# aras-p/ToyPathTracer

Measured on AMD Instinct MI355X. Metric: Mray/s, higher is better.
Workload: dtype f32

## Files before the change

include/tpt_test_hooks.h:

```cpp
#ifndef TPT_TEST_HOOKS_H
#define TPT_TEST_HOOKS_H
#include "tpt_hip.h"
#ifdef __cplusplus
extern "C" {
#endif
TPT_API int tptTestMath(int op, const float* a, const float* b, float* out, int n);
TPT_API int tptTestHitSpheres(int hitSpheres, const float* rays, int* outId, float* outT, int n);
TPT_API int tptTestMathExhaustive(int op, unsigned lo, unsigned hi, unsigned long long* outMismatches, unsigned* outFirst8);
TPT_API int tptTestMatrixFilter(const float* rays, unsigned long long* outMask, int* outId, float* outT, int n);
TPT_API int tptTestGroupFilter(const float* rays, int n, unsigned long long* outViolations, unsigned long long* outTouched, unsigned long long* outExact);
TPT_API int tptTestSetDealCapacities(int superGroupEntries, int groupEntries, int survivorEntries);
TPT_API int tptDebugStats(unsigned long long* out128, int reset);
TPT_API int tptDebugChunkOrder(unsigned* outCost, unsigned* outOrder, int capacity);
#ifdef __cplusplus
}
#endif
#endif
```

toypathtracer_amd/api.py:

```python
import ctypes as C
import os

import numpy as np

kFlagAnimate = 1 << 0
kFlagProgressive = 1 << 1
SEED_ROW_SERIAL, SEED_PER_PIXEL = 0, 1
FOLD_RECURSIVE, FOLD_FORWARD = 0, 1

SPHERE_DT = np.dtype([("cx", "<f4"), ("cy", "<f4"), ("cz", "<f4"), ("radius", "<f4"), ("invRadius", "<f4")])
MATERIAL_DT = np.dtype([("type", "<i4"), ("albedo", "<f4", 3), ("emissive", "<f4", 3), ("roughness", "<f4"), ("ri", "<f4")])
CAMERA_DT = np.dtype([("origin", "<f4", 3), ("lowerLeftCorner", "<f4", 3), ("horizontal", "<f4", 3), ("vertical", "<f4", 3),
                      ("uu", "<f4", 3), ("vv", "<f4", 3), ("ww", "<f4", 3), ("lensRadius", "<f4")])


class TptError(RuntimeError):
    pass


_lib = None
_product = None
_hooks = None

C_ABI_SYMBOLS = [
    "tptInitialize", "tptShutdown", "tptUpdate", "tptDraw", "tptGetObjectCount", "tptGetSceneDesc",
    "tptSetSamplesPerPixel", "tptSetConfig", "tptSetSeedMode", "tptSetFoldMode", "tptSetScene", "tptSetCamera", "tptSetStream",
    "tptSetRowShard", "tptLocalRowCount", "tptLocalRowToGlobal", "tptDrawDevice", "tptRayCounterRead", "tptSetRayCounter", "tptSetFrameOverlap", "tptDisplayRGBA8", "tptKernelTimingBegin", "tptKernelTimingEnd",
    "tptSynchronize", "tptTimerBegin", "tptTimerEnd", "tptSetKernelVariant",
    "tptDrawDeviceBatch", "tptDrawDeviceViews", "tptDrawDeviceAnimation", "tptDrawDeviceAov", "tptDenoiseDevice", "tptDrawDeviceMoments", "tptDrawDeviceAnimationMoments", "tptDrawDeviceCameraClip", "tptDrawDeviceKeyframeClip", "tptDenoiseDeviceVariance", "tptTemporalAccumulateDevice", "tptObjectPlaneDevice", "tptObjectMotionTable", "tptTemporalAccumulateObjectsDevice", "tptDenoiseClipDevice", "tptMotionVectorsDevice", "tptRectifyHistoryDevice", "tptDrawDeviceAdaptive", "tptAdaptiveSamplesDevice", "tptDrawShardedBatch", "tptGetLookaheadHits", "tptCommGetUniqueId", "tptCommInit", "tptCommInitLoopback", "tptCommInfo", "tptCommDestroy", "tptDrawSharded", "tptSetShardExchangeInterval", "tptShardedFinish", "tptGetLaunchInfo", "tptGetPipelineInfo", "tptGetSceneInfo", "tptSetHostBufferMode", "tptSetHostLookahead", "tptSetStreamBatching", "tptSetTileMirror", "tptGetLastError", "tptSetErrorHandler", "tptGetDeviceName",
]
HOOK_SYMBOLS = ["tptTestMath", "tptTestMathExhaustive", "tptTestHitSpheres", "tptTestMatrixFilter", "tptTestGroupFilter", "tptTestSetDealCapacities", "tptDebugStats", "tptDebugChunkOrder"]
CXX_ABI_SYMBOLS = [
    "_Z14InitializeTestv", "_Z12ShutdownTestv", "_Z10UpdateTestfiiij", "_Z8DrawTestfiiiPfRij",
    "_Z14GetObjectCountRiS_S_S_", "_Z12GetSceneDescPvS_S_S_Pi",
]


class ClipDenoiseArgs(C.Structure):
    _fields_ = ([("screenWidth", C.c_int), ("screenHeight", C.c_int), ("nFrames", C.c_int), ("clipFlags", C.c_uint)]
                + [(name, C.c_void_p) for name in ("deviceFrameImages", "deviceFrameMoments", "deviceFrameAlbedo", "deviceFrameNormalDepth",
                                                   "cameras", "deviceFrameObjects", "deviceFrameObjectMotion", "deviceFrameOut",
                                                   "prevCamera", "devicePrevNormalDepth", "devicePrevObject", "deviceHistory")]
                + [("nObjects", C.c_int), ("iterations", C.c_int), ("denoiseFlags", C.c_uint)]
                + [(name, C.c_float) for name in ("samples", "sigmaLuminance", "sigmaNormal", "sigmaDepth", "maxHistory", "depthTolerance",
                                                  "normalTolerance", "coverageTolerance")])


class MotionVectorsArgs(C.Structure):
    _fields_ = ([("screenWidth", C.c_int), ("screenHeight", C.c_int), ("nFrames", C.c_int), ("flags", C.c_uint)]
                + [(name, C.c_void_p) for name in ("cameras", "deviceFrameAlbedo", "deviceFrameNormalDepth", "deviceFrameObjects",
                                                   "deviceFrameObjectMotion", "deviceFrameMotion", "prevCamera", "devicePrevAlbedo",
                                                   "devicePrevNormalDepth", "devicePrevObject")]
                + [("nObjects", C.c_int)]
                + [(name, C.c_float) for name in ("depthTolerance", "normalTolerance", "coverageTolerance")])


def _lib_dir():
    return os.environ.get("TPT_LIB_DIR") or os.path.join(os.path.dirname(os.path.abspath(__file__)), "lib")


def library_path():
    return os.environ.get("TPT_LIB") or os.path.join(_lib_dir(), "libtoypathtracer_hip.so")


def hooks_library_path():
    return os.environ.get("TPT_LIB") or os.path.join(_lib_dir(), "libtoypathtracer_hip_hooks.so")


def _bind(path, hooks):
    lib = C.CDLL(path)
    i, f, u, p = C.c_int, C.c_float, C.c_uint, C.c_void_p
    sigs = {
        "tptInitialize": [], "tptShutdown": [], "tptUpdate": [f, i, i, i, u],
        "tptDraw": [f, i, i, i, p, C.POINTER(i), u],
        "tptGetObjectCount": [C.POINTER(i)] * 4, "tptGetSceneDesc": [p, p, p, p, C.POINTER(i)],
        "tptSetSamplesPerPixel": [i], "tptSetConfig": [i, f, i], "tptSetSeedMode": [i], "tptSetFoldMode": [i], "tptSetScene": [p, p, i],
        "tptSetCamera": [p, p, f, f, f], "tptSetStream": [p], "tptSetRowShard": [i, i, i], "tptLocalRowCount": [i],
        "tptLocalRowToGlobal": [i], "tptDrawDevice": [f, i, i, i, p, u], "tptRayCounterRead": [C.POINTER(C.c_int64)],
        "tptSetRayCounter": [p], "tptSetTileMirror": [p, p], "tptSetFrameOverlap": [i], "tptDisplayRGBA8": [p, i, i, p], "tptKernelTimingBegin": [i],
        "tptKernelTimingEnd": [C.POINTER(f), C.POINTER(i)],
        "tptSynchronize": [], "tptTimerBegin": [], "tptTimerEnd": [C.POINTER(f)], "tptSetKernelVariant": [i, i, i],
        "tptGetLaunchInfo": [C.POINTER(i)] * 4, "tptGetPipelineInfo": [C.POINTER(i)] * 4, "tptGetSceneInfo": [C.POINTER(i)] * 3, "tptCommGetUniqueId": [p], "tptCommInit": [p, i, i, i], "tptCommInitLoopback": [i, i], "tptCommInfo": [C.POINTER(i)] * 3, "tptCommDestroy": [], "tptDrawSharded": [f, i, i, i, p, u], "tptSetShardExchangeInterval": [i], "tptDrawShardedBatch": [f, i, i, i, i, p, u], "tptDrawDeviceBatch": [f, i, i, i, i, p, u], "tptDrawDeviceViews": [f, i, i, i, i, p, p, p, u], "tptDrawDeviceAnimation": [i, i, p, i, i, p, p, p, u], "tptDrawDeviceAov": [f, i, i, i, p, p, p, u], "tptDenoiseDevice": [i, i, p, p, p, p, i, f, f, f, u], "tptDrawDeviceMoments": [f, i, i, i, p, p, p, p, u], "tptDrawDeviceAnimationMoments": [i, i, p, i, i] + [p] * 7 + [u], "tptDrawDeviceCameraClip": [i, i, p, p, i, i] + [p] * 8 + [u], "tptDrawDeviceKeyframeClip": [i, i, p, i, p, p, i, i] + [p] * 9 + [u], "tptDenoiseDeviceVariance": [i, i, p, p, p, p, f, p, i, f, f, f, u], "tptTemporalAccumulateDevice": [i, i] + [p] * 14 + [f] * 4, "tptObjectPlaneDevice": [i, p, p, i, i, p, u], "tptObjectMotionTable": [f, f, u, p, i], "tptTemporalAccumulateObjectsDevice": [i, i] + [p] * 14 + [f] * 4 + [p, p, p, i], "tptDenoiseClipDevice": [C.POINTER(ClipDenoiseArgs)], "tptMotionVectorsDevice": [C.POINTER(MotionVectorsArgs)], "tptRectifyHistoryDevice": [i, i] + [p] * 7 + [i, f], "tptDrawDeviceAdaptive": [f, i, i, i, p, p, p, p, p, u], "tptAdaptiveSamplesDevice": [i, i, p, f, i, i, p, p, p], "tptShardedFinish": [C.POINTER(C.c_int64)], "tptSetHostBufferMode": [i], "tptGetLookaheadHits": [C.POINTER(C.c_longlong)], "tptSetHostLookahead": [i], "tptSetStreamBatching": [i],
    }
    if hooks:
        sigs.update({"tptDebugStats": [p, i], "tptDebugChunkOrder": [p, p, i], "tptTestMath": [i, p, p, p, i], "tptTestMathExhaustive": [i, u, u, p, p],
                     "tptTestHitSpheres": [i, p, p, p, i], "tptTestMatrixFilter": [p, p, p, p, i], "tptTestGroupFilter": [p, i, p, p, p], "tptTestSetDealCapacities": [i, i, i]})
    for name, args in sigs.items():
        fn = getattr(lib, name)
        fn.argtypes = args
        fn.restype = i
    lib.tptGetLastError.restype = C.c_char_p
    lib.tptGetDeviceName.restype = C.c_char_p
    return lib


def _preload():
    try:
        import torch
    except ImportError:
        pass


def load_library():
    global _lib, _product
    if _lib is not None:
        return _lib
    _preload()
    path = library_path()
    if not os.path.exists(path):
        raise TptError(f"{path} is missing: build it with `python -c 'import __graft_entry__ as g; g.build()'` "
                       "(toypathtracer_amd/csrc/build.sh). There is no CPU fallback.")
    _product = _bind(path, hooks=bool(os.environ.get("TPT_LIB")) and _has_hooks(path))
    _lib = _product
    return _lib


def _has_hooks(path):
    try:
        return hasattr(C.CDLL(path), "tptTestMath")
# ... 835 lines not shown


def test_hit_spheres(rays, hit_spheres=0):
    rays = np.ascontiguousarray(rays, np.float32).reshape(-1, 6)
    n = rays.shape[0]
    ids = np.empty(n, np.int32)
    ts = np.empty(n, np.float32)
    _chk(_hook("tptTestHitSpheres")(hit_spheres, rays.ctypes.data, ids.ctypes.data, ts.ctypes.data, n),
         "tptTestHitSpheres")
    return ids, ts


def test_matrix_filter(rays, hits=False):
    rays = np.ascontiguousarray(rays, np.float32).reshape(-1, 6)
    n = rays.shape[0]
    masks = np.empty(n, np.uint64)
    ids = np.empty(n, np.int32) if hits else None
    ts = np.empty(n, np.float32) if hits else None
    _chk(_hook("tptTestMatrixFilter")(rays.ctypes.data, masks.ctypes.data, ids.ctypes.data if hits else None,
                                            ts.ctypes.data if hits else None, n), "tptTestMatrixFilter")
    return (masks, ids, ts) if hits else masks


def test_set_deal_capacities(super_group_entries=0, group_entries=0, survivor_entries=0):
    _chk(_hook("tptTestSetDealCapacities")(super_group_entries, group_entries, survivor_entries), "tptTestSetDealCapacities")


def test_group_filter(rays):
    rays = np.ascontiguousarray(rays, np.float32).reshape(-1, 6)
    n = rays.shape[0]
    v = [C.c_ulonglong(0) for _ in range(3)]
    _chk(_hook("tptTestGroupFilter")(rays.ctypes.data, n, C.byref(v[0]), C.byref(v[1]), C.byref(v[2])), "tptTestGroupFilter")
    return int(v[0].value), v[1].value / n, v[2].value / n
```

toypathtracer_amd/csrc/tpt_context.h:

```cpp
#pragma once
#include "../../include/tpt_hip.h"
#if defined(TPT_TEST_HOOKS)
#include "../../include/tpt_test_hooks.h"
#endif
#include "../../include/tpt_test_api.h"
#include "tpt_device.h"
#include "tpt_queue_layout.h"
#include "tpt_scene.h"
#include "tpt_shard.h"
#include "tpt_stream_batch.h"
#include "tpt_animation.h"
#include <hip/hip_runtime.h>
#include <thread>
#include <rccl/rccl.h>
#include <chrono>
#include <dlfcn.h>
#include <map>
#include <stdio.h>
#include <stdlib.h>
#include <string>


namespace tpth {
using namespace tpt;

const int kMaxBatch = 32;
static_assert(kMaxBatch == TPT_Q_VIEWS_MAX, "a batch's cameras, centres and ray counts have their places in the path-queue kernel's LDS");
struct TraceTicket {
    int slot = 0, nPixels = 0;
    bool pipelined = false, valid = false;
    float lerpFac = 0;
    const f4* colour = nullptr;
    int batch = 1;
    tptLerpTable lerp = {};
    const f4* moments = nullptr;
    TraceTicket plane(int j) const
    {
        TraceTicket t = *this;
        t.colour = colour + (size_t)j * (size_t)nPixels;
        if (batch > 1) t.lerpFac = lerp.v[j];
        t.batch = 1;
        return t;
    }
};

struct Streak {
    int frame = 0, w = 0, h = 0, n = 0;
    unsigned flags = 0;
    unsigned long long key = 0;
    int next(int frame_, int w_, int h_, unsigned flags_, unsigned long long key_)
    {
        n = frame_ == frame + 1 && w_ == w && h_ == h && flags_ == flags && key_ == key ? n + 1 : 0;
        frame = frame_; w = w_; h = h_; flags = flags_; key = key_;
        return n;
    }
};

struct PendingLaunch {
    enum Kind { AHEAD, ROW_SERIAL, STREAM } kind = AHEAD;
    TraceTicket T;
    int firstFrame = 0, next = 0;
    int w = 0, h = 0;
    unsigned flags = 0;
    unsigned long long key = 0;
    unsigned long long* rays = nullptr;
};
struct LaunchQueue {
    static const int kCap = 4;
    PendingLaunch e[kCap];
    int n = 0;
    bool empty() const { return n == 0; }
    bool holds(PendingLaunch::Kind kind) const { return n > 0 && e[0].kind == kind; }
    bool frontMatches(PendingLaunch::Kind kind, int frame, int w, int h, unsigned flags, unsigned long long key) const;
    void serveFront(bool wasOpen, TraceTicket& T, const unsigned long long*& rays);
    int push(const PendingLaunch& L);
    int discard();
    void closeStream();
};

struct Context {
    static const int kMaxOverlap = 16;
    static const int kMaxSlots = 2 * kMaxOverlap;
    static const int kOrderTables = kMaxSlots + 2;
    bool inited = false;
    int device = 0, numCUs = 0;
    int traceCUs = 0;
    std::string deviceName, err;
    hipStream_t ownStream = nullptr, stream = nullptr;
    hipEvent_t ev0 = nullptr, ev1 = nullptr;

    std::vector<SpherePOD> spheres;
    std::vector<MaterialPOD> mats;
    CameraSetup camSetup = defaultCameraSetup();
    CameraPOD cam;
    PackedScene packed;
    bool sceneDirty = true;
    bool updated = false;
    int updatedW = 0, updatedH = 0;

    static const int kSceneSets = 2 * kMaxSlots;
    struct SceneSet {
        char* dev = nullptr;
        char* stage = nullptr;
        size_t cap = 0, bytes = 0;
        size_t offSph4 = 0, offInvR = 0, offMats = 0, offLights = 0;
        size_t offGPairs = 0, offGSph = 0, offGId = 0, offBSph = 0, offBId = 0;
        size_t offSPairs = 0;
        int nSuperPairs = 0;
        size_t offAmat = 0;
        int mxR1 = -1;
// ... 34 lines not shown
    long long lastTotal = 0;

    f4* dStack[kMaxSlots] = {};
    size_t stackCap = 0, colourCap = 0;
    int slotsReserved = 0;
    int smallStreak = 0;
    int slotReservations = 0;
    unsigned* dChunkCost = nullptr;
    unsigned* dChunkOrder[kOrderTables] = {};
    unsigned* dChunkSnap[kMaxOverlap] = {};
    int chunkCap = 0, chunkCount = 0;
    int costOrder = 1;
    hipEvent_t evOrder = nullptr;
    hipStream_t orderStream = nullptr;
    unsigned long long orderSeq = 0;
    int lastOrderTable = 0;
    float* dFrame = nullptr;
    hipStream_t hostStream2 = nullptr;
    hipEvent_t evBand = nullptr, evBandEnd = nullptr;
    int hostTrust = 0;
    const float* tileSrc = nullptr;
    int tileW = 0, tileH = 0;
    int lookahead = 2;
    LaunchQueue pending;
    struct HostCaller {
        Streak seq;
        int refusedW = 0, refusedH = 0;
        unsigned long long refusedKey = 0;
    } hostCaller;
    static const int kStreamBatchMax = 8, kStreamRing = 64;
    unsigned long long streamBatches = 0;
    int streamRun = 0, streamNext = -1;
    int streamBatch = 1;
    struct DeviceCaller {
        int lastSlot = -1, syncStreak = 0;
        Streak seq;
    } devCaller;
    struct ViewSlot {
        CameraPOD* dev = nullptr;
        unsigned long long* rays = nullptr;
        CameraPOD* stage = nullptr;
        hipEvent_t evUploaded = nullptr;
        bool copyEnqueued = false;
    } views[kMaxSlots];
    char* dViews = nullptr;
    CameraPOD* hViewsStage = nullptr;
    f4* dAovSums = nullptr;
    size_t aovSumsBytes = 0;
    hipEvent_t evAov = nullptr;
    f4* dMoments = nullptr;
    size_t momentsBytes = 0;
    hipEvent_t evClip[2] = {nullptr, nullptr};
    unsigned clipSeq = 0;
    f4* dKeySph = nullptr;
    f4* hKeySph = nullptr;
    size_t keySphBytes = 0;
    hipEvent_t evKeySph[2] = {nullptr, nullptr};
    bool keySphCopied[2] = {false, false};
    unsigned keySphSeq = 0;
    f4* dDenoise = nullptr;
    size_t denoiseBytes = 0;
    f4* dClipStage = nullptr;
    size_t clipStageBytes = 0;
    tptFlowConsts* dFlowConsts = nullptr;
    tptFlowConsts* hFlowConsts = nullptr;
    size_t flowConstsBytes = 0;
// ... 145 lines not shown
```

toypathtracer_amd/csrc/tpt_device.h:

```cpp
#pragma once
#include "tpt_trace.h"
#include "tpt_frame_pools.h"

#ifndef TPT_BLOCK
#define TPT_BLOCK 64
#endif
#define TPT_CHUNK_PIXELS 256

namespace tpt {

struct KernelArgs {
    SceneView scene;
    FrameConsts fc;
    f4* frameColour;
    int nLocalRows, stripeRows, stripeStride, stripeOffset;
    int tilesX;
    int numItems;
    int numChunks, chunkSize;
    int batchFrames, chunksPerFrame, framePlane;
    unsigned totalWaves;
    int laneCap;
    int noRefill;
    f4* stackBuf;
    int stackStride;
    int ldsStackLevels;
    f4* pathBuf;
    const unsigned* chunkOrder;
    unsigned* chunkCost;
    int chunkShift;
    unsigned* work;
    unsigned long long* rayCounter;
    int rayCounterStride;
    unsigned gen;
    int helperBase;
    int helperPct;
    int ldsGroupPairs;
    const CameraPOD* viewCams = nullptr;
    const f4* moveCentres = nullptr;
    f4* aovSums = nullptr;
    f4* aovAlbedo = nullptr;
    f4* aovNormalDepth = nullptr;
    f4* momentsOut = nullptr;
    int aovPlane = 0;
    const int32_t* sampleCounts = nullptr;
    const f4* keyCentres = nullptr;
    unsigned long long keyMask = 0;
    int keyCount = 0;
    int framePools = 0;
};

}

hipError_t tptLaunchTrace(const tpt::KernelArgs& a, int hs, int fold, bool ldsScene, int blocks, size_t lds, hipStream_t stream);
int tptTraceOccupancy(int hs, int fold, bool ldsScene, size_t lds);
hipError_t tptLaunchTraceQueue(const tpt::KernelArgs& a, bool ldsScene, int blocks, size_t lds, hipStream_t stream);
int tptQueueMatrixFilter();
int tptQueueGroupMatrixBounds();
hipError_t tptLaunchDisplay(const float* tile, unsigned char* rgba, int width, int height, hipStream_t stream);
__attribute__((weak)) hipError_t tptLaunchDenoise(const float* colour, const float* albedo, const float* normalDepth, float* out,
                                                  float* scratch, int width, int height, int iterations, float ic, float in, float id,
                                                  bool demodulate, hipStream_t stream);
__attribute__((weak)) hipError_t tptLaunchDenoiseVariance(const float* colour, const float* albedo, const float* normalDepth,
                                                          const float* moments, float* out, float* scratch, int width, int height,
                                                          int iterations, float samples, float sl2, float in, float id, bool demodulate,
                                                          hipStream_t stream);
__attribute__((weak)) hipError_t tptLaunchFramesAtrous(const float* colour, const float* albedo, const float* normalDepth,
                                                       const float* moments, float* out, float* scratch, int width, int height, int frames,
                                                       int iterations, float samples, float sl2, float in, float id, bool demodulate,
                                                       hipStream_t stream);
struct tptTemporalConsts {
    float o[3], ll[3], H[3], V[3];
    float po[3], pa[3], pw[3], pH[3], pV[3];
    float pf, phh, pvv;
    float maxHistory, depthTol, normalTol, coverageTol;
};
__attribute__((weak)) hipError_t tptLaunchTemporal(const float* colour, const float* albedo, const float* normalDepth, const float* moments,
                                                   const float* prevColour, const float* prevAlbedo, const float* prevNormalDepth,
                                                   const float* prevMoments, float* outColour, float* outAlbedo, float* outMoments,
                                                   float* outVariance, int width, int height, const tptTemporalConsts& k,
                                                   hipStream_t stream);
struct tptObjectPlaneConsts {
// ... 53 lines not shown
```

toypathtracer_amd/csrc/tpt_frame_pools.h:

```cpp
#pragma once

#if defined(__HIPCC__)
#define TPT_FP_HD __host__ __device__ inline
#else
#define TPT_FP_HD inline
#endif

namespace tpt {

const int kFramePoolBase = 4;
const int kFramePoolsMax = 8;

TPT_FP_HD int framePoolsOfLaunch(int batch, int blocks, bool plain, bool helpable)
{
    return (plain && !helpable && batch >= 2 && batch <= kFramePoolsMax && blocks >= 2 * batch) ? batch : 0;
}

TPT_FP_HD unsigned framePoolOfBlock(unsigned block, unsigned pools, unsigned blocks)
{
    return block * pools / blocks;
}

}
```

toypathtracer_amd/csrc/tpt_host.cpp:

```cpp
#include "tpt_context.h"

using namespace tpt;
using namespace tpth;

namespace tpth {

Context g;

int localRows(int h) { return shardLocalRows(h, g.stripeRows, g.numParts, g.part); }
int localToGlobal(int ly) { return shardLocalToGlobal(ly, g.stripeRows, g.numParts, g.part); }

template <class T>
int ensureDev(T*& p, int& cap, int need)
{
    if (need <= cap && p) return 0;
    if (p) HIPCHK(hipFree(p));
    p = nullptr;
    int n = need < 64 ? 64 : need;
    HIPCHK(hipMalloc(reinterpret_cast<void**>(&p), sizeof(T) * (size_t)n));
    cap = n;
    return 0;
}

size_t align256(size_t v) { return (v + 255) & ~(size_t)255; }
// ... 249 lines not shown
    hipDeviceProp_t prop;
    HIPCHK(hipGetDeviceProperties(&prop, dev));
    g.device = dev;
    g.numCUs = prop.multiProcessorCount;
    g.deviceName = std::string(prop.name) + " (" + prop.gcnArchName + ")";
    HIPCHK(hipStreamCreateWithFlags(&g.ownStream, hipStreamDefault));
    g.stream = g.ownStream;
    HIPCHK(hipEventCreateWithFlags(&g.evOrder, kOrderingEvent));
    HIPCHK(hipEventCreate(&g.ev0));
    HIPCHK(hipEventCreate(&g.ev1));
    HIPCHK(hipMalloc(reinterpret_cast<void**>(&g.dWork), 64 * Context::kMaxSlots));
    HIPCHK(hipMemsetAsync(g.dWork, 0, 64 * Context::kMaxSlots, g.stream));
    {
        int rc = createTraceStreams();
        if (rc) return rc;
    }
    for (int k = 0; k < Context::kMaxSlots; ++k) {
        HIPCHK(hipEventCreateWithFlags(&g.evTrace[k], kOrderingEvent));
        HIPCHK(hipEventCreateWithFlags(&g.evResolve[k], kOrderingEvent));
        g.resolveRecorded[k] = false;
    }

    g.frameSeq = 0;
    g.oldestPending = 0;
    HIPCHK(hipStreamCreateWithFlags(&g.hostStream2, hipStreamNonBlocking));
    HIPCHK(hipEventCreateWithFlags(&g.evBand, kOrderingEvent));
    HIPCHK(hipEventCreateWithFlags(&g.evBandEnd, kOrderingEvent));
    const size_t pendingRays = sizeof(unsigned long long) * (Context::kMaxSlots + 2 * kMaxBatch + Context::kStreamRing * Context::kStreamBatchMax);
    HIPCHK(hipMalloc(reinterpret_cast<void**>(&g.dRaysAhead), pendingRays));
    HIPCHK(hipMemsetAsync(g.dRaysAhead, 0, pendingRays, g.stream));
    g.dRaysBatch = g.dRaysAhead + Context::kMaxSlots;
    g.dRaysStream = g.dRaysBatch + 2 * kMaxBatch;
    g.pending.n = 0;
    if (const char* esb = getenv("TPT_STREAM_BATCH")) g.streamBatch = atoi(esb) != 0;
    HIPCHK(hipMalloc(reinterpret_cast<void**>(&g.dRaysOwn), 64));
    HIPCHK(hipMemsetAsync(g.dRaysOwn, 0, 64, g.stream));
    HIPCHK(hipStreamSynchronize(g.stream));
    g.dRays = g.dRaysOwn;
    g.lastTotal = 0;
    if (g.spheres.empty()) defaultScene(g.spheres, g.mats);
    if (const char* e6 = getenv("TPT_GRID_FILL")) g.gridFill = atoi(e6);
    if (const char* e7 = getenv("TPT_HOST_PACE")) g.hostPace = atoi(e7);
    if (const char* eh = getenv("TPT_TAIL_HELPERS")) g.helpersOn = atoi(eh) != 0;
    for (int k = 0; k < Context::kMaxSlots; ++k) {
        HIPCHK(hipEventCreateWithFlags(&g.evPre[k], kOrderingEvent));
        g.hrec[k].valid = false;
    }
    g.launchGen = 0;
    if (const char* e5 = getenv("TPT_GRID_DIV")) g.gridDiv = atoi(e5) > 0 ? atoi(e5) : 0;
    g.sceneDirty = true;
    {
        int rc = probeHardwareQueues();
        if (rc) return rc;
    }
    g.inited = true;
    return 0;
}

int tptShutdown(void)
{
    if (!g.inited) return 0;
    (void)g.pending.discard();
    (void)tptCommDestroy();
    (void)hipStreamSynchronize(g.stream);
    (void)hipDeviceSynchronize();
    for (int k = 0; k < Context::kMaxSlots; ++k) {
// ... 37 lines not shown
        if (g.views[k].evUploaded) (void)hipEventDestroy(g.views[k].evUploaded);
        g.views[k] = Context::ViewSlot();
    }
    (void)hipFree(g.dViews); g.dViews = nullptr;
    (void)hipFree(g.dAovSums); g.dAovSums = nullptr;
    g.aovSumsBytes = 0;
    if (g.evAov) { (void)hipEventDestroy(g.evAov); g.evAov = nullptr; }
    for (hipEvent_t& e : g.evClip)
        if (e) { (void)hipEventDestroy(e); e = nullptr; }
    (void)hipFree(g.dMoments); g.dMoments = nullptr;
    g.momentsBytes = 0;
    (void)hipFree(g.dKeySph); g.dKeySph = nullptr;
    if (g.hKeySph) (void)hipHostFree(g.hKeySph);
    g.hKeySph = nullptr;
    g.keySphBytes = 0;
    for (int i = 0; i < 2; ++i) {
        g.keySphCopied[i] = false;
        if (g.evKeySph[i]) { (void)hipEventDestroy(g.evKeySph[i]); g.evKeySph[i] = nullptr; }
    }
    (void)hipFree(g.dDenoise); g.dDenoise = nullptr;
    g.denoiseBytes = 0;
    (void)hipFree(g.dClipStage); g.dClipStage = nullptr;
    g.clipStageBytes = 0;
    (void)hipFree(g.dFlowConsts); g.dFlowConsts = nullptr;
    if (g.hFlowConsts) (void)hipHostFree(g.hFlowConsts);
    g.hFlowConsts = nullptr;
    g.flowConstsBytes = 0;
    for (int i = 0; i < 2; ++i) {
        g.flowCopied[i] = false;
        if (g.evFlow[i]) { (void)hipEventDestroy(g.evFlow[i]); g.evFlow[i] = nullptr; }
    }
    if (g.hViewsStage) (void)hipHostFree(g.hViewsStage);
    g.hViewsStage = nullptr;
    g.inited = false;
    g.updated = false;
    g.updatedW = g.updatedH = 0;
    g.occCache.clear();
    g.mirror = nullptr; g.mirrorCounter = nullptr;
    if (g.hostStream2) { (void)hipStreamSynchronize(g.hostStream2); (void)hipStreamDestroy(g.hostStream2); g.hostStream2 = nullptr; }
    if (g.evBand) { (void)hipEventDestroy(g.evBand); g.evBand = nullptr; }
    if (g.evBandEnd) { (void)hipEventDestroy(g.evBandEnd); g.evBandEnd = nullptr; }
    g.tileSrc = nullptr; g.tileW = g.tileH = 0;
    g.pending.n = 0;
    (void)hipFree(g.dRaysAhead); g.dRaysAhead = g.dRaysBatch = g.dRaysStream = nullptr;
    g.orderStream = nullptr; g.oldestPending = 0; g.frameSeq = 0;
    g.streamDepth = 1; g.prevInFlight = -1;
    g.hostCaller = Context::HostCaller(); g.devCaller = Context::DeviceCaller();
    g.smallStreak = 0; g.configEpoch = 1;
    return 0;
}

int tptSetStream(void* hipStream)
{
    if (int rc_ = flushShardDeferred()) return rc_;
    if (requireInit()) return -1;
    if (g.pending.discard()) return -2;
    HIPCHK(hipStreamSynchronize(g.stream));
    g.stream = hipStream ? reinterpret_cast<hipStream_t>(hipStream) : g.ownStream;
    return 0;
}

int tptSetSamplesPerPixel(int spp)
{
    if (int rc_ = flushShardDeferred()) return rc_;
    if (spp < 1 || spp > 65536) return fail("tptSetSamplesPerPixel: spp out of range");
    if (spp == g.spp) return 0;
// ... 280 lines not shown
```

toypathtracer_amd/csrc/tpt_host_draw.cpp:

```cpp
#include "tpt_context.h"

using namespace tpt;
using namespace tpth;

namespace tpth {

bool LaunchQueue::frontMatches(PendingLaunch::Kind kind, int frame, int w, int h, unsigned flags, unsigned long long key) const
{
    const PendingLaunch& F = e[0];
    return holds(kind) && frame == F.firstFrame + F.next && F.w == w && F.h == h && F.flags == flags && F.key == key;
}

void LaunchQueue::serveFront(bool wasOpen, TraceTicket& T, const unsigned long long*& rays)
{
    PendingLaunch& F = e[0];
    if (wasOpen && F.kind != PendingLaunch::STREAM) g.aheadHits++;
    T = F.T.plane(F.next);
    rays = F.rays + F.next;
    if (++F.next < F.T.batch) return;
    for (int k = 0; k + 1 < n; ++k) e[k] = e[k + 1];
    --n;
}

int LaunchQueue::push(const PendingLaunch& L)
{
    if (n == kCap || (n > 0 && !holds(L.kind))) return fail("internal: launch queue full or of another kind");
    e[n++] = L;
    return 0;
}

int LaunchQueue::discard()
{
    if (n > 0 && !holds(PendingLaunch::STREAM))
        for (int k = 0; k < Context::kMaxOverlap; ++k) HIPCHK(hipStreamSynchronize(g.traceStream[k]));
    n = 0;
    return 0;
}

void LaunchQueue::closeStream()
{
    if (holds(PendingLaunch::STREAM)) n = 0;
    g.streamNext = -1;
}

int traceAhead(int frameCount, int w, int h, unsigned testFlags, unsigned long long key, int want)
{
    LaunchQueue& Q = g.pending;
    int nextFrame = Q.n ? Q.e[Q.n - 1].firstFrame + 1 : frameCount + 1;
    const int nSlots = effectiveOverlap();
    const int maxAhead = want < nSlots - 2 ? want : nSlots - 2;
    while (Q.n < maxAhead) {
        PendingLaunch A;
        A.firstFrame = nextFrame++; A.w = w; A.h = h; A.flags = testFlags; A.key = key;
        A.rays = g.dRaysAhead + g.frameSeq % (unsigned long long)Context::kMaxSlots;
        int rc = enqueueTrace(A.firstFrame, w, h, testFlags, A.rays, A.T);
        if (rc) return rc;
        if (!A.T.valid) break;
        if ((rc = Q.push(A))) return rc;
    }
    return 0;
}

static int checkDenoise(const char* fn, bool variance, int w, int h, const float* colour, const float* albedo, const float* normalDepth,
                        const float* moments, const float* out, int iterations, float samples, float sigma0, float sigmaNormal,
                        float sigmaDepth, unsigned flags)
{
    const std::string f(fn);
    if (w < 1 || w > 8192 || h < 1 || h > 8192) return fail(f + ": w and h must lie in 1..8192");
    if (!colour || !out) return fail(f + ": deviceColour and deviceOut are required");
    if (variance && !moments) return fail(f + ": deviceMoments is required");
    if (overlapsAny(out, {colour, albedo, normalDepth, moments}, (uintptr_t)w * (uintptr_t)h * 16u)) return fail(f + ": deviceOut overlaps an input");
    if (iterations < 1 || iterations > 8) return fail(f + ": iterations must lie in 1..8");
    auto sigmaOk = [](float s) { return s == 0.0f || (s >= 1e-6f && s <= 1e6f); };
// ... 712 lines not shown
```

toypathtracer_amd/csrc/tpt_host_hooks.cpp:

```cpp
#include "tpt_context.h"

using namespace tpt;
using namespace tpth;

extern "C" {
#if defined(TPT_TEST_HOOKS)
int tptDebugChunkOrder(unsigned* outCost, unsigned* outOrder, int capacity)
{
    if (requireInit()) return -1;
    HIPCHK(hipStreamSynchronize(g.stream));
    for (int k = 0; k < Context::kMaxOverlap; ++k) HIPCHK(hipStreamSynchronize(g.traceStream[k]));
    int n = g.chunkCount < capacity ? g.chunkCount : capacity;
    if (n <= 0 || !g.dChunkCost) return 0;
    if (outCost) HIPCHK(hipMemcpy(outCost, g.dChunkCost, sizeof(unsigned) * n, hipMemcpyDeviceToHost));
    if (outOrder) HIPCHK(hipMemcpy(outOrder, g.dChunkOrder[g.lastOrderTable], sizeof(unsigned) * n, hipMemcpyDeviceToHost));
    return n;
}

int tptDebugStats(unsigned long long* out64, int reset)
{
    if (requireInit()) return -1;
    HIPCHK(hipStreamSynchronize(g.stream));
    int rc = out64 ? tptReadStats(out64) : 0;
    if (rc == -1) return fail("tptDebugStats: library not built with -DTPT_STATS (profiling build, tools/build_stats.sh)");
// ... 119 lines not shown
        return fail("tptTestSetDealCapacities: each size between 64 and its compiled value, or 0, 0, 0 for the compiled ones");
    return 0;
}

int tptTestHitSpheres(int hitSpheres, const float* rays, int* outId, float* outT, int n)
{
    if (requireInit()) return -1;
    if (!rays || !outId || !outT || n <= 0) return fail("tptTestHitSpheres: bad arguments");
    if (g.sceneDirty || (g.curSet < 0 && g.pendingSet < 0)) {
        int rc = stageScene();
        if (rc) return rc;
    }
    {
        int rc = enqueueSceneUpload(g.stream);
        if (rc) return rc;
    }
    float *dr = nullptr, *dt = nullptr;
    int* di = nullptr;
    HIPCHK(hipMalloc(reinterpret_cast<void**>(&dr), sizeof(float) * 6 * n));
    HIPCHK(hipMalloc(reinterpret_cast<void**>(&dt), sizeof(float) * n));
    HIPCHK(hipMalloc(reinterpret_cast<void**>(&di), sizeof(int) * n));
    HIPCHK(hipMemcpy(dr, rays, sizeof(float) * 6 * n, hipMemcpyHostToDevice));
    KernelArgs a;
    memset(&a, 0, sizeof(a));
    a.scene = deviceView();
    HIPCHK(tptLaunchHitTest(a, hitSpheres == 1 ? HS_SIMPLE : HS_TWO_PHASE, dr, di, dt, n, g.stream));
    HIPCHK(hipStreamSynchronize(g.stream));
    HIPCHK(hipMemcpy(outId, di, sizeof(int) * n, hipMemcpyDeviceToHost));
    HIPCHK(hipMemcpy(outT, dt, sizeof(float) * n, hipMemcpyDeviceToHost));
    (void)hipFree(dr); (void)hipFree(dt); (void)hipFree(di);
    return 0;
}

#endif
}
```

toypathtracer_amd/csrc/tpt_host_pipeline.cpp:

```cpp
#include "tpt_context.h"

using namespace tpt;
using namespace tpth;

namespace tpth {

struct FramePlan {
    KernelArgs a;
    bool rowSerial = false, queued = false, ldsScene = false, useOrder = false;
    size_t lds = 0;
    int occ = 0, threadsPerBlock = 0, blocks = 0;
    int nOverlap = 1;
    int nSlots = 1, slot = 0;
    int batch = 1;
    bool plainFrame = true;
    const char* entry = "tptDrawDevice";
};

int syncAllStreams();
int reserveSlotBuffers(int nSlots, size_t colourBytes, size_t stackBytes)
{
    const bool small = colourBytes * 4 <= g.colourCap && g.colourCap * (size_t)g.slotsReserved > (1ull << 30);
    g.smallStreak = small ? g.smallStreak + 1 : 0;
    const bool shrink = small && g.smallStreak >= 8 && g.pending.empty();
// ... 505 lines not shown
            (void)hipGetLastError();
        }
        HIPCHK(hipStreamWaitEvent(ts, g.evResolve[slot], 0));
    }
    if ((rc = enqueueSceneUpload(ts))) return rc;
    if (aov && ts != g.stream) {
        if (clip) {
            const unsigned h = g.clipSeq & 1u;
            HIPCHK(hipEventRecord(g.evClip[h ^ 1u], g.stream));
            HIPCHK(hipStreamWaitEvent(ts, aov->continues ? g.evClip[h] : g.evClip[h ^ 1u], 0));
        } else {
            HIPCHK(hipEventRecord(g.evAov, g.stream));
            HIPCHK(hipStreamWaitEvent(ts, g.evAov, 0));
        }
    }
    if (clip) g.clipSeq++;
    if (viewCams || centres || keyCentres) {
        static_assert(2 * sizeof(f4) * kMaxBatch <= sizeof(CameraPOD) * kMaxBatch, "a batch's moving centres fit the slot's camera table");
        Context::ViewSlot& V = g.views[slot];
        const f4* behind = keyCentres ? keyCentres : centres;
        const size_t camBytes = sizeof(CameraPOD) * (size_t)batch, centreBytes = (keyCentres ? (size_t)TPT_Q_KEYS_MAX : 2) * sizeof(f4) * (size_t)batch;
        const size_t bytes = viewCams && behind ? kViewCamBytes + centreBytes : (viewCams ? camBytes : centreBytes);
        if (V.copyEnqueued) HIPCHK(hipEventSynchronize(V.evUploaded));
        if (viewCams) memcpy(V.stage, viewCams, camBytes);
        if (behind) memcpy(reinterpret_cast<char*>(V.stage) + (viewCams ? kViewCamBytes : 0), behind, centreBytes);
        HIPCHK(hipMemcpyAsync(V.dev, V.stage, bytes, hipMemcpyHostToDevice, ts));
        HIPCHK(hipEventRecord(V.evUploaded, ts));
        V.copyEnqueued = true;
    }
    if ((rc = enqueueChunkOrder(P, ts))) return rc;
    if (frameRays && frameRays != g.dRays) HIPCHK(hipMemsetAsync(frameRays, 0, sizeof(unsigned long long) * (size_t)(rayStride > 0 ? batch : 1), ts));
    const bool helpable = P.queued && pipelined && batch == 1 && !P.rowSerial && !table && !aov;
    a.framePools = framePoolsOfLaunch(batch, P.blocks, P.queued && !P.rowSerial && !table && !aov, helpable);
    a.helperBase = 0;
    a.helperPct = 0;
    a.gen = 0u;
    g.hrec[slot].valid = false;
    if (helpable) {
        if (++g.launchGen == 0u) g.launchGen = 1u;
        a.gen = g.launchGen;
        HIPCHK(hipEventRecord(g.evPre[slot], ts));
    }
    const bool timeIt = g.kernelTiming && g.ktUsed < g.ktStart.size();
    if (timeIt) HIPCHK(hipEventRecord(g.ktStart[g.ktUsed], ts));
    if (P.queued)
        HIPCHK(tptLaunchTraceQueue(a, P.ldsScene, P.blocks, P.lds, ts));
    else
        HIPCHK(tptLaunchTrace(a, g.hs, g.foldMode, P.ldsScene, P.blocks, P.lds, ts));
    seqGuard.launched = true;
    if (timeIt) {
        HIPCHK(hipEventRecord(g.ktStop[g.ktUsed], ts));
        g.ktUsed++;
    }
    if (pipelined) HIPCHK(hipEventRecord(g.evTrace[slot], ts));
    if (helpable) {
        Context::HelperRec& R = g.hrec[slot];
        R.a = a; R.ldsScene = P.ldsScene; R.blocks = P.blocks; R.maxBlocks = maxGridBlocks(P); R.lds = P.lds;
        R.helped = false; R.valid = true; R.ts = ts;
    }
    T.slot = slot;
    T.nPixels = a.nLocalRows * w;
    T.pipelined = pipelined;
    T.lerpFac = a.fc.lerpFac;
    T.colour = a.frameColour;
    T.moments = a.momentsOut;
    T.batch = batch;
// ... 316 lines not shown
    D.syncStreak = prevDone ? D.syncStreak + 1 : 0;
    const int seqStreak = D.seq.next(frameCount, w, h, testFlags, key);
    const bool lookAhead = pipelined && stable && !g.mirror && g.lookahead > 0 && D.syncStreak >= 2 && seqStreak >= 2;

    LaunchQueue& Q = g.pending;
    TraceTicket T;
    const unsigned long long* rays = nullptr;
    int rc;
    const bool hit = stable && !g.mirror && Q.frontMatches(PendingLaunch::AHEAD, frameCount, w, h, testFlags, key);
    if (!hit && !lookAhead) {
        if (stable && Q.frontMatches(PendingLaunch::STREAM, frameCount, w, h, testFlags, key)) {
            Q.serveFront(true, T, rays);
        } else {
            const bool continues = Q.empty() && seqStreak >= 2 && frameCount == g.streamNext;
            if ((rc = Q.discard())) return rc;
            g.streamNext = -1;
            int nBatch = 1;
            if (g.streamBatch && pipelined && stable && seqStreak >= 2 && pathQueueTakesScene() && w <= 8192 && h <= 8192) {
                g.streamRun = continues ? g.streamRun + 1 : 0;
                nBatch = streamBatchFrames((long long)localRows(h) * w * g.spp, effectiveOverlap(), Context::kMaxOverlap, g.streamRun,
                                           (long long)localRows(h) * w * (long long)sizeof(f4), Context::kStreamBatchMax);
            }
            if (nBatch > 1) {
                PendingLaunch S;
                S.kind = PendingLaunch::STREAM;
                S.firstFrame = frameCount; S.w = w; S.h = h; S.flags = testFlags; S.key = key;
                S.rays = g.dRaysStream + (g.streamBatches % (unsigned long long)Context::kStreamRing) * Context::kStreamBatchMax;
                rc = enqueueTrace(frameCount, w, h, testFlags, S.rays, S.T, nBatch, 1);
                if (rc == kRefused && localRows(h) * (long long)w * g.spp >= kStreamLaunchSamples) {
                    nBatch = 1;
                } else if (rc) {
                    return rc;
                } else if (S.T.valid) {
                    g.streamBatches++;
                    g.streamNext = frameCount + nBatch;
                    if ((rc = Q.push(S))) return rc;
                    Q.serveFront(false, T, rays);
                }
            }
            if (nBatch == 1 && (rc = enqueueTrace(frameCount, w, h, testFlags, nullptr, T)))
                return rc;
        }
        rc = enqueueResolve(T, deviceTile, rays);
        if (T.valid) D.lastSlot = T.slot;
        return rc;
    }
    const int devAhead = g.lookahead + 1 < 3 ? g.lookahead + 1 : 3;
    DepthScope depthScope(1 + devAhead);
    if (hit) {
        Q.serveFront(true, T, rays);
    } else {
        if ((rc = Q.discard())) return rc;
        unsigned long long* own = g.dRaysAhead + g.frameSeq % (unsigned long long)Context::kMaxSlots;
        if ((rc = enqueueTrace(frameCount, w, h, testFlags, own, T))) return rc;
        rays = T.valid ? own : nullptr;
    }
    if (lookAhead && T.valid && (rc = traceAhead(frameCount, w, h, testFlags, key, devAhead))) return rc;
    rc = enqueueResolve(T, deviceTile, rays);
    if (T.valid) D.lastSlot = T.slot;
    return rc;
}

int tptDrawDeviceBatch(float time, int firstFrame, int nFrames, int w, int h, float* deviceTile, unsigned testFlags)
{
    (void)time;
    if (int rc_ = flushShardDeferred()) return rc_;
// ... 192 lines not shown
    if (int rc_ = flushShardDeferred()) return rc_;
    if (requireInit()) return -1;
    if (g.pending.discard()) return -2;
    HIPCHK(hipStreamSynchronize(g.stream));
    g.dRays = deviceU64 ? static_cast<unsigned long long*>(deviceU64) : g.dRaysOwn;
    int64_t total = 0;
    int rc = tptRayCounterRead(&total);
    if (rc) return rc;
    g.lastTotal = total;
    return 0;
}

int tptSynchronize(void)
{
    if (int rc_ = flushShardDeferred()) return rc_;
    if (requireInit()) return -1;
    g.pending.closeStream();
    if (int rc = launchTailHelpers()) return rc;
    HIPCHK(hipStreamSynchronize(g.stream));
    return 0;
}

int tptTimerBegin(void)
{
    if (requireInit()) return -1;
    HIPCHK(hipEventRecord(g.ev0, g.stream));
    return 0;
}
int tptTimerEnd(float* outMs)
{
    if (int rc_ = flushShardDeferred()) return rc_;
    if (requireInit()) return -1;
    HIPCHK(hipEventRecord(g.ev1, g.stream));
    if (int rc = launchTailHelpers()) return rc;
    HIPCHK(hipEventSynchronize(g.ev1));
    float ms = 0;
    HIPCHK(hipEventElapsedTime(&ms, g.ev0, g.ev1));
    if (outMs) *outMs = ms;
    return 0;
}

}
```

toypathtracer_amd/csrc/tpt_kernels.hip:

```cpp
#include "../../include/tpt_hip.h"
#include "tpt_device.h"
#include "tpt_queue_layout.h"
#include "tpt_shard.h"

namespace tpt {

__device__ __forceinline__ unsigned waveReduceAdd(unsigned v)
{
#pragma unroll
    for (int off = 32; off > 0; off >>= 1) v += __shfl_down(v, off, 64);
    return v;
}

__device__ __forceinline__ void storeColour(const KernelArgs& a, const Lane& L)
{
    f3 c = lanePixelColour(L, a.fc);
    f4 v;
    v.x = c.x; v.y = c.y; v.z = c.z; v.w = 0.0f;
    a.frameColour[L.pix] = v;
}

__global__ void __launch_bounds__(256) tptResolveKernel(float* __restrict__ tile, const f4* __restrict__ colour, int nPixels, float lerpFac,
                                                        const unsigned long long* frameRays, unsigned long long* totalRays)
{
// ... 1611 lines not shown
    for (int i = tid; i < a.scene.nLights * 2; i += TPT_Q_T) ldsLights[i] = a.scene.lights[i];
    sv.lights = ldsLights;
    float* ldsGpairs = reinterpret_cast<float*>(smem + ((off + 15) & ~15));
    if (!LDS_SCENE && a.ldsGroupPairs > 0)
        for (int i = tid; i < a.ldsGroupPairs * 8; i += TPT_Q_T) ldsGpairs[(i / TPT_GPAIR_FLOATS) * TPT_GPAIR_LDS_STRIDE + (i % TPT_GPAIR_FLOATS)] = a.scene.gpairs[i];
#if TPT_MATRIX_FILTER
    if (useMatrix)
        for (int i = tid; i < TPT_MXH_TABLE_DWORDS; i += TPT_Q_T) ldsA[i] = a.scene.amatH[i];
    const int mxR1 = a.scene.mxR1;
#endif
#if defined(__HIP_DEVICE_COMPILE__) && defined(TPT_STATS) && TPT_STATS >= 2
    if (tid < 4) g_hsLds[tid] = 0ull;
#if TPT_GROUP_DEAL
    if (tid < 18) g_dealLds[tid] = 0ull;
#endif
#endif
    for (int i = tid; i < (int)(sizeof(FrameConsts) / 4); i += TPT_Q_T) reinterpret_cast<uint32_t*>(ldsFc)[i] = reinterpret_cast<const uint32_t*>(&a.fc)[i];
    if (CAM_TABLE)
        for (int i = tid; i < a.batchFrames * (int)(sizeof(CameraPOD) / 4); i += TPT_Q_T)
            reinterpret_cast<uint32_t*>(ldsCams)[i] = reinterpret_cast<const uint32_t*>(a.viewCams)[i];
    if (MOVING)
        for (int i = tid; i < a.batchFrames * kMovedPerFrame; i += TPT_Q_T) ldsMoved[i] = KEYS ? a.keyCentres[i] : a.moveCentres[i];
    const uint64_t keyMask = KEYS ? (uint64_t)a.keyMask : 0ull;
    for (int i = tid; i < Q_COUNT * TPT_Q_P; i += TPT_Q_T) q[i] = (unsigned short)(i < kPaths ? i : 0xFFFF);
    if (tid < 8) {
        ctl->head[tid] = 0u;
        ctl->tail[tid] = tid == Q_FREE ? (unsigned)kPaths : 0u;
    }
    if (tid == 0) {
        ctl->poolTotal = 0u;
        ctl->globalExhausted = 0u;
    }
    if (BATCH && tid < 32) ctl->frameRays[tid] = 0u;
    __syncthreads();

    const FrameConsts& fc = a.fc;
    const unsigned long long laneBelow = (1ull << lane) - 1ull;
#if TPT_MATRIX_FILTER
    SceneView svM = sv;
    svM.sph4 = ldsSphFixed;
#endif
#if TPT_GROUP_DEAL
    LdsList dealList = (LdsList)(smem + kOffDeal + (tid >> 6) * TPT_GROUP_DEAL_WAVE_BYTES);
    unsigned* dealCount = reinterpret_cast<unsigned*>(smem + kOffDeal + (tid >> 6) * TPT_GROUP_DEAL_WAVE_BYTES + TPT_GROUP_DEAL_ENTRIES * 4);
    const bool groupDeal = !MOVING && !LDS_SCENE && sv.nGroups > 0 && sv.nGroups <= 65536;
#endif
    f4* colSum = st + 2 * kPaths;
    int chunkNext = 0, chunkEnd = 0;
    int chunkFrame = 0;
    bool noMoreChunks = false;
    unsigned myRays = 0;
    auto poolFrame = [&]() { return framePoolOfBlock(blockIdx.x, (unsigned)uniformHere(a.batchFrames), (unsigned)uniformHere((int)gridDim.x)); };
#if defined(TPT_STATS)
    const unsigned long long qT0 = wall_clock64();
    unsigned qSteps = 0, qBatches = 0, qIdle = 0;
    unsigned long long qSec[5] = {0, 0, 0, 0, 0};
#endif

#if defined(TPT_STATS)
#define TPT_TSTAMP(v)                      \
    __builtin_amdgcn_sched_barrier(0);     \
    __builtin_amdgcn_s_waitcnt(0);         \
    const unsigned long long v = __builtin_amdgcn_s_memtime(); \
    __builtin_amdgcn_sched_barrier(0)
#if TPT_STATS < 2
#define TPT_TADD(slot, a, b) do { if (lane == 0) atomicAdd(&g_tptStats[slot], (b) - (a)); } while (0)
#else
#define TPT_TADD(slot, a, b) do { qSec[(slot) == 64 + 24 ? 4 : ((slot) & 3)] += (b) - (a); } while (0)
#endif
#else
#define TPT_TSTAMP(v) do { } while (0)
#define TPT_TADD(slot, a, b) do { } while (0)
#endif
    for (;;) {
        TPT_TSTAMP(tsTop);
        unsigned myAvail = 0, myHead = 0, myTail = 0;
        if (lane < Q_COUNT) {
            myTail = __hip_atomic_load(&ctl->tail[lane], __ATOMIC_RELAXED, __HIP_MEMORY_SCOPE_WORKGROUP);
            myHead = __hip_atomic_load(&ctl->head[lane], __ATOMIC_RELAXED, __HIP_MEMORY_SCOPE_WORKGROUP);
            myAvail = myTail - myHead;
        }
        unsigned avail[Q_COUNT];
#pragma unroll
        for (int c = 0; c < Q_COUNT; ++c) avail[c] = (unsigned)__builtin_amdgcn_readlane((int)myAvail, c);
        const bool canStart = (chunkEnd > chunkNext) || !noMoreChunks;
// ... 976 lines not shown
```

Baseline: 45590.

## Let host cut a streamed batch so blocks skip frames no longer needed

Adds a host-visible pinned cut word per launch slot. The host writes it when a streamed frame batch is closed or cut at the front, recording how many frames are still wanted. At kernel start each pooled block reads the word with a system-scope atomic load and remaps itself onto one of the kept frames, so work on discarded speculative frames is skipped. The cost is one extra system-memory read per block, a change in how blocks are assigned to frame pools, and reuse of frameRays[0] in LDS as the frame index. It also adds test hooks to preset a cut and read back per-frame ray counts.

New measurement: 49790, median of 6. +9.2%, better.

```diff
diff --git a/include/tpt_test_hooks.h b/include/tpt_test_hooks.h
--- a/include/tpt_test_hooks.h
+++ b/include/tpt_test_hooks.h
@@ -12,6 +12,8 @@
 TPT_API int tptTestSetDealCapacities(int superGroupEntries, int groupEntries, int survivorEntries);
 TPT_API int tptDebugStats(unsigned long long* out128, int reset);
 TPT_API int tptDebugChunkOrder(unsigned* outCost, unsigned* outOrder, int capacity);
+TPT_API int tptTestPresetStreamCut(int keep);
+TPT_API int tptTestStreamFrameRays(unsigned long long* outRays, int capacity);
 #ifdef __cplusplus
 }
 #endif
diff --git a/toypathtracer_amd/api.py b/toypathtracer_amd/api.py
--- a/toypathtracer_amd/api.py
+++ b/toypathtracer_amd/api.py
@@ -29,7 +29,7 @@
     "tptSynchronize", "tptTimerBegin", "tptTimerEnd", "tptSetKernelVariant",
     "tptDrawDeviceBatch", "tptDrawDeviceViews", "tptDrawDeviceAnimation", "tptDrawDeviceAov", "tptDenoiseDevice", "tptDrawDeviceMoments", "tptDrawDeviceAnimationMoments", "tptDrawDeviceCameraClip", "tptDrawDeviceKeyframeClip", "tptDenoiseDeviceVariance", "tptTemporalAccumulateDevice", "tptObjectPlaneDevice", "tptObjectMotionTable", "tptTemporalAccumulateObjectsDevice", "tptDenoiseClipDevice", "tptMotionVectorsDevice", "tptRectifyHistoryDevice", "tptDrawDeviceAdaptive", "tptAdaptiveSamplesDevice", "tptDrawShardedBatch", "tptGetLookaheadHits", "tptCommGetUniqueId", "tptCommInit", "tptCommInitLoopback", "tptCommInfo", "tptCommDestroy", "tptDrawSharded", "tptSetShardExchangeInterval", "tptShardedFinish", "tptGetLaunchInfo", "tptGetPipelineInfo", "tptGetSceneInfo", "tptSetHostBufferMode", "tptSetHostLookahead", "tptSetStreamBatching", "tptSetTileMirror", "tptGetLastError", "tptSetErrorHandler", "tptGetDeviceName",
 ]
-HOOK_SYMBOLS = ["tptTestMath", "tptTestMathExhaustive", "tptTestHitSpheres", "tptTestMatrixFilter", "tptTestGroupFilter", "tptTestSetDealCapacities", "tptDebugStats", "tptDebugChunkOrder"]
+HOOK_SYMBOLS = ["tptTestMath", "tptTestMathExhaustive", "tptTestHitSpheres", "tptTestMatrixFilter", "tptTestGroupFilter", "tptTestSetDealCapacities", "tptDebugStats", "tptDebugChunkOrder", "tptTestPresetStreamCut", "tptTestStreamFrameRays"]
 CXX_ABI_SYMBOLS = [
     "_Z14InitializeTestv", "_Z12ShutdownTestv", "_Z10UpdateTestfiiij", "_Z8DrawTestfiiiPfRij",
     "_Z14GetObjectCountRiS_S_S_", "_Z12GetSceneDescPvS_S_S_Pi",
@@ -84,7 +84,7 @@
     }
     if hooks:
         sigs.update({"tptDebugStats": [p, i], "tptDebugChunkOrder": [p, p, i], "tptTestMath": [i, p, p, p, i], "tptTestMathExhaustive": [i, u, u, p, p],
-                     "tptTestHitSpheres": [i, p, p, p, i], "tptTestMatrixFilter": [p, p, p, p, i], "tptTestGroupFilter": [p, i, p, p, p], "tptTestSetDealCapacities": [i, i, i]})
+                     "tptTestHitSpheres": [i, p, p, p, i], "tptTestMatrixFilter": [p, p, p, p, i], "tptTestGroupFilter": [p, i, p, p, p], "tptTestSetDealCapacities": [i, i, i], "tptTestPresetStreamCut": [i], "tptTestStreamFrameRays": [p, i]})
     for name, args in sigs.items():
         fn = getattr(lib, name)
         fn.argtypes = args
@@ -986,3 +986,15 @@
     v = [C.c_ulonglong(0) for _ in range(3)]
     _chk(_hook("tptTestGroupFilter")(rays.ctypes.data, n, C.byref(v[0]), C.byref(v[1]), C.byref(v[2])), "tptTestGroupFilter")
     return int(v[0].value), v[1].value / n, v[2].value / n
+
+
+def test_preset_stream_cut(keep):
+    _chk(_hook("tptTestPresetStreamCut")(int(keep)), "tptTestPresetStreamCut")
+
+
+def test_stream_frame_rays():
+    out = np.zeros(8, np.uint64)
+    n = _hook("tptTestStreamFrameRays")(out.ctypes.data, 8)
+    if n < 0:
+        raise TptError(f"tptTestStreamFrameRays: {_lib.tptGetLastError().decode()}")
+    return [int(v) for v in out[:n]]
diff --git a/toypathtracer_amd/csrc/tpt_context.h b/toypathtracer_amd/csrc/tpt_context.h
--- a/toypathtracer_amd/csrc/tpt_context.h
+++ b/toypathtracer_amd/csrc/tpt_context.h
@@ -34,6 +34,7 @@
     int batch = 1;
     tptLerpTable lerp = {};
     const f4* moments = nullptr;
+    unsigned cutSerial = 0;
     TraceTicket plane(int j) const
     {
         TraceTicket t = *this;
@@ -76,6 +77,7 @@
     int push(const PendingLaunch& L);
     int discard();
     void closeStream();
+    void cutFront();
 };
 
 struct Context {
@@ -176,6 +178,11 @@
     unsigned long long streamBatches = 0;
     int streamRun = 0, streamNext = -1;
     int streamBatch = 1;
+    unsigned* hCut = nullptr;
+    unsigned cutSerial = 0;
+    int cutPreset = 0;
+    unsigned long long* lastStreamRays = nullptr;
+    int lastStreamFrames = 0;
     struct DeviceCaller {
         int lastSlot = -1, syncStreak = 0;
         Streak seq;
diff --git a/toypathtracer_amd/csrc/tpt_device.h b/toypathtracer_amd/csrc/tpt_device.h
--- a/toypathtracer_amd/csrc/tpt_device.h
+++ b/toypathtracer_amd/csrc/tpt_device.h
@@ -47,6 +47,8 @@
     unsigned long long keyMask = 0;
     int keyCount = 0;
     int framePools = 0;
+    const unsigned* cutWord = nullptr;
+    unsigned cutSerial = 0;
 };
 
 }
diff --git a/toypathtracer_amd/csrc/tpt_frame_pools.h b/toypathtracer_amd/csrc/tpt_frame_pools.h
--- a/toypathtracer_amd/csrc/tpt_frame_pools.h
+++ b/toypathtracer_amd/csrc/tpt_frame_pools.h
@@ -21,4 +21,23 @@
     return block * pools / blocks;
 }
 
+TPT_FP_HD unsigned frameCutWord(unsigned serial, unsigned keep)
+{
+    return serial << 8 | (keep & 0xffu);
 }
+TPT_FP_HD unsigned frameCutNextSerial(unsigned serial)
+{
+    return (serial & 0xffffffu) == 0xffffffu ? 1u : (serial & 0xffffffu) + 1u;
+}
+TPT_FP_HD unsigned framesKeptUnderCut(unsigned word, unsigned serial, unsigned pools)
+{
+    const unsigned keep = word - (serial << 8);
+    return (serial != 0u && keep - 1u < pools - 1u) ? keep : pools;
+}
+TPT_FP_HD unsigned frameServedUnderCut(unsigned block, unsigned pools, unsigned blocks, unsigned keep)
+{
+    const unsigned own = framePoolOfBlock(block, pools, blocks);
+    return own < keep ? own : block % keep;
+}
+
+}
diff --git a/toypathtracer_amd/csrc/tpt_host.cpp b/toypathtracer_amd/csrc/tpt_host.cpp
--- a/toypathtracer_amd/csrc/tpt_host.cpp
+++ b/toypathtracer_amd/csrc/tpt_host.cpp
@@ -305,6 +305,9 @@
     g.dRaysBatch = g.dRaysAhead + Context::kMaxSlots;
     g.dRaysStream = g.dRaysBatch + 2 * kMaxBatch;
     g.pending.n = 0;
+    HIPCHK(hipHostMalloc(reinterpret_cast<void**>(&g.hCut), sizeof(unsigned) * Context::kMaxSlots, hipHostMallocDefault));
+    memset(g.hCut, 0, sizeof(unsigned) * Context::kMaxSlots);
+    g.cutSerial = 0; g.cutPreset = 0; g.lastStreamRays = nullptr; g.lastStreamFrames = 0;
     if (const char* esb = getenv("TPT_STREAM_BATCH")) g.streamBatch = atoi(esb) != 0;
     HIPCHK(hipMalloc(reinterpret_cast<void**>(&g.dRaysOwn), 64));
     HIPCHK(hipMemsetAsync(g.dRaysOwn, 0, 64, g.stream));
@@ -408,6 +411,9 @@
     }
     if (g.hViewsStage) (void)hipHostFree(g.hViewsStage);
     g.hViewsStage = nullptr;
+    if (g.hCut) (void)hipHostFree(g.hCut);
+    g.hCut = nullptr;
+    g.lastStreamRays = nullptr; g.lastStreamFrames = 0;
     g.inited = false;
     g.updated = false;
     g.updatedW = g.updatedH = 0;
diff --git a/toypathtracer_amd/csrc/tpt_host_draw.cpp b/toypathtracer_amd/csrc/tpt_host_draw.cpp
--- a/toypathtracer_amd/csrc/tpt_host_draw.cpp
+++ b/toypathtracer_amd/csrc/tpt_host_draw.cpp
@@ -33,12 +33,22 @@
 {
     if (n > 0 && !holds(PendingLaunch::STREAM))
         for (int k = 0; k < Context::kMaxOverlap; ++k) HIPCHK(hipStreamSynchronize(g.traceStream[k]));
+    cutFront();
     n = 0;
     return 0;
 }
 
+void LaunchQueue::cutFront()
+{
+    if (!holds(PendingLaunch::STREAM) || !g.hCut) return;
+    const PendingLaunch& F = e[0];
+    if (F.T.valid && F.T.cutSerial != 0u && F.next >= 1 && F.next < F.T.batch)
+        __atomic_store_n(g.hCut + F.T.slot, frameCutWord(F.T.cutSerial, (unsigned)F.next), __ATOMIC_RELEASE);
+}
+
 void LaunchQueue::closeStream()
 {
+    cutFront();
     if (holds(PendingLaunch::STREAM)) n = 0;
     g.streamNext = -1;
 }
diff --git a/toypathtracer_amd/csrc/tpt_host_hooks.cpp b/toypathtracer_amd/csrc/tpt_host_hooks.cpp
--- a/toypathtracer_amd/csrc/tpt_host_hooks.cpp
+++ b/toypathtracer_amd/csrc/tpt_host_hooks.cpp
@@ -175,5 +175,24 @@
     return 0;
 }
 
+int tptTestPresetStreamCut(int keep)
+{
+    if (requireInit()) return -1;
+    if (keep < 0 || keep >= Context::kStreamBatchMax) return fail("tptTestPresetStreamCut: keep must lie in 0..7 (0: no preset)");
+    g.cutPreset = keep;
+    return 0;
+}
+
+int tptTestStreamFrameRays(unsigned long long* outRays, int capacity)
+{
+    if (requireInit()) return -1;
+    if (int rc = tptSynchronize()) return rc;
+    for (int k = 0; k < Context::kMaxOverlap; ++k) HIPCHK(hipStreamSynchronize(g.traceStream[k]));
+    const int n = g.lastStreamFrames < capacity ? g.lastStreamFrames : capacity;
+    if (n <= 0 || !g.lastStreamRays || !outRays) return 0;
+    HIPCHK(hipMemcpy(outRays, g.lastStreamRays, sizeof(unsigned long long) * (size_t)n, hipMemcpyDeviceToHost));
+    return n;
+}
+
 #endif
 }
diff --git a/toypathtracer_amd/csrc/tpt_host_pipeline.cpp b/toypathtracer_amd/csrc/tpt_host_pipeline.cpp
--- a/toypathtracer_amd/csrc/tpt_host_pipeline.cpp
+++ b/toypathtracer_amd/csrc/tpt_host_pipeline.cpp
@@ -561,6 +561,17 @@
     if (frameRays && frameRays != g.dRays) HIPCHK(hipMemsetAsync(frameRays, 0, sizeof(unsigned long long) * (size_t)(rayStride > 0 ? batch : 1), ts));
     const bool helpable = P.queued && pipelined && batch == 1 && !P.rowSerial && !table && !aov;
     a.framePools = framePoolsOfLaunch(batch, P.blocks, P.queued && !P.rowSerial && !table && !aov, helpable);
+    a.cutWord = nullptr;
+    a.cutSerial = 0u;
+    T.cutSerial = 0u;
+    if (a.framePools > 0) {
+        g.cutSerial = frameCutNextSerial(g.cutSerial);
+        a.cutWord = g.hCut + slot;
+        a.cutSerial = g.cutSerial;
+        T.cutSerial = g.cutSerial;
+        __atomic_store_n(g.hCut + slot, g.cutPreset > 0 ? frameCutWord(g.cutSerial, (unsigned)g.cutPreset) : 0u, __ATOMIC_RELEASE);
+        g.cutPreset = 0;
+    }
     a.helperBase = 0;
     a.helperPct = 0;
     a.gen = 0u;
@@ -943,6 +954,8 @@
                 } else if (rc) {
                     return rc;
                 } else if (S.T.valid) {
+                    g.lastStreamRays = S.rays;
+                    g.lastStreamFrames = nBatch;
                     g.streamBatches++;
                     g.streamNext = frameCount + nBatch;
                     if ((rc = Q.push(S))) return rc;
@@ -1201,6 +1214,7 @@
     if (int rc_ = flushShardDeferred()) return rc_;
     if (requireInit()) return -1;
     HIPCHK(hipEventRecord(g.ev1, g.stream));
+    g.pending.closeStream();
     if (int rc = launchTailHelpers()) return rc;
     HIPCHK(hipEventSynchronize(g.ev1));
     float ms = 0;
diff --git a/toypathtracer_amd/csrc/tpt_kernels.hip b/toypathtracer_amd/csrc/tpt_kernels.hip
--- a/toypathtracer_amd/csrc/tpt_kernels.hip
+++ b/toypathtracer_amd/csrc/tpt_kernels.hip
@@ -1667,6 +1667,12 @@
         ctl->globalExhausted = 0u;
     }
     if (BATCH && tid < 32) ctl->frameRays[tid] = 0u;
+    if (POOLS && tid == 0) {
+        typedef const __attribute__((address_space(1))) unsigned* GlobalWord;
+        const unsigned pools = (unsigned)a.batchFrames;
+        const unsigned word = __hip_atomic_load((GlobalWord)a.cutWord, __ATOMIC_RELAXED, __HIP_MEMORY_SCOPE_SYSTEM);
+        ctl->frameRays[0] = frameServedUnderCut(blockIdx.x, pools, gridDim.x, framesKeptUnderCut(word, a.cutSerial, pools));
+    }
     __syncthreads();
 
     const FrameConsts& fc = a.fc;
@@ -1685,7 +1691,7 @@
     int chunkFrame = 0;
     bool noMoreChunks = false;
     unsigned myRays = 0;
-    auto poolFrame = [&]() { return framePoolOfBlock(blockIdx.x, (unsigned)uniformHere(a.batchFrames), (unsigned)uniformHere((int)gridDim.x)); };
+    auto poolFrame = [&]() { return (unsigned)__builtin_amdgcn_readfirstlane((int)ctl->frameRays[0]); };
 #if defined(TPT_STATS)
     const unsigned long long qT0 = wall_clock64();
     unsigned qSteps = 0, qBatches = 0, qIdle = 0;
```
